# ywyue/AGILE3D

Measured on AMD Instinct MI355X. Metric: scenes/s (80k-voxel, 10 clicks), higher is better.
Workload: dtype f32; 1 GPU; batch of 16 synthetic 79736-voxel scenes, 10 clicks each (5 objects x 2), scene build + forward_backbone + 1 forward_mask per scene, fp32, eval; voxels=79736, queries=20, parallelism=scene-sharded x1 (no data-path collective), global_batch=16, steps_in_flight_per_gpu=4

## Files before the change

### agile3d_amd/csrc/spconv.hip

```cpp
#include "common.h"
#include <stdlib.h>

namespace a3d {

typedef float f32x4 __attribute__((ext_vector_type(4)));

struct ConvArgs {
  const float* in;
  int ldi, n_in;
  const int* nbr;
  int nbr_stride;
  const uint32_t* gmask;
  const float* w;
  int K, cin, cout;
  float* out;
  int ldo, n_out;
  const int* out_map;
  const float* scale;
  const float* shift;
  const float* res;
  int ldr;
  int relu;
  int zero_row;
  int tag_table, tag_level;
// ... 1071 lines not shown
  return A3D_OK;
}

template <int NS, int NCT, bool HAS2>
__global__ void __launch_bounds__(768) k_dense(const float* __restrict__ X, int ldx, const float* __restrict__ X2,
                                                   int ldx2, int n, const float* __restrict__ Wp,
                                                   const float* __restrict__ scale, const float* __restrict__ shift,
                                                   const float* __restrict__ res, int ldr, int relu,
                                                   float* __restrict__ Y, int ldy, int ngroups, int zero_row,
                                                   const int* __restrict__ out_map) {
  extern __shared__ __attribute__((aligned(16))) char smem[];
  f32x4* Wl = (f32x4*)smem;
  if (zero_row >= 0 && blockIdx.x == 0 && threadIdx.x < 16 * NCT) Y[(size_t)zero_row * ldy + threadIdx.x] = 0.f;
  const int lane = threadIdx.x & 63, wave = threadIdx.x >> 6;
  const int g = lane >> 4, j = lane & 15;
  const int nw = blockDim.x >> 6;
  const int stride = gridDim.x * nw;
  int grp = blockIdx.x * nw + wave;
  f32x4 nx[NS], nx2[HAS2 ? NS : 1];
  auto fetch = [&](int gq) {
    const int row = min(gq * 16 + j, n - 1);
    const float* xr = X + (size_t)row * ldx + 4 * g;
#pragma unroll
    for (int S = 0; S < NS; ++S) nx[S] = *(const f32x4*)(xr + 16 * S);
    if constexpr (HAS2) {
      const float* x2r = X2 + (size_t)row * ldx2 + 4 * g;
#pragma unroll
      for (int S = 0; S < NS; ++S) nx2[S] = *(const f32x4*)(x2r + 16 * S);
    }
  };
  if (grp < ngroups) fetch(grp);
  {
    constexpr int TOT = NS * NCT * 64;
    const int bd = blockDim.x;
    for (int base = threadIdx.x; base < TOT; base += 8 * bd) {
      f32x4 t8[8];
#pragma unroll
      for (int u = 0; u < 8; ++u)
        if (base + u * bd < TOT) t8[u] = ((const f32x4*)Wp)[base + u * bd];
#pragma unroll
      for (int u = 0; u < 8; ++u)
        if (base + u * bd < TOT) Wl[base + u * bd] = t8[u];
    }
  }
  __syncthreads();
  while (grp < ngroups) {
    f32x4 a[NS];
#pragma unroll
    for (int S = 0; S < NS; ++S) {
      if constexpr (HAS2) a[S] = nx[S] + nx2[S];
      else a[S] = nx[S];
    }
    const int next = grp + stride;
    if (next < ngroups) fetch(next);
    f32x4 acc[NCT];
#pragma unroll
    for (int ct = 0; ct < NCT; ++ct) acc[ct] = (f32x4){0.f, 0.f, 0.f, 0.f};
    {
      static_assert(NCT % 2 == 0, "pairs of 16-column tiles");
      constexpr int NP = NS * NCT / 2;
      const f32x4* Ws = Wl + lane;
      f32x4 c0 = Ws[0], c1 = Ws[64];
#pragma unroll
      for (int pi = 0; pi < NP; ++pi) {
        const int S = pi / (NCT / 2), ct = 2 * (pi % (NCT / 2));
        f32x4 n0 = c0, n1 = c1;
        if (pi + 1 < NP) {
          n0 = Ws[(2 * pi + 2) * 64];
          n1 = Ws[(2 * pi + 3) * 64];
        }
        __builtin_amdgcn_sched_barrier(0);
#pragma unroll
        for (int t = 0; t < 4; ++t) {
          acc[ct] = __builtin_amdgcn_mfma_f32_16x16x4f32(c0[t], a[S][t], acc[ct], 0, 0, 0);
          acc[ct + 1] = __builtin_amdgcn_mfma_f32_16x16x4f32(c1[t], a[S][t], acc[ct + 1], 0, 0, 0);
        }
        __builtin_amdgcn_sched_barrier(0);
        c0 = n0;
        c1 = n1;
      }
    }
    if (grp * 16 + j < n) {
      const int row = out_map ? out_map[grp * 16 + j] : grp * 16 + j;
#pragma unroll
      for (int ct = 0; ct < NCT; ++ct) {
        const int col = 16 * ct + 4 * g;
        f32x4 v = acc[ct];
        if (scale) v *= *(const f32x4*)(scale + col);
        if (shift) v += *(const f32x4*)(shift + col);
        if (res) v += *(const f32x4*)(res + (size_t)row * ldr + col);
        if (relu) {
#pragma unroll
          for (int t = 0; t < 4; ++t) v[t] = fmaxf(v[t], 0.f);
        }
        *(f32x4*)(Y + (size_t)row * ldy + col) = v;
      }
    }
    grp = next;
  }
}

static void allow_big_lds();
static bool dense_supported(int cin, int cout) {
  return (cin == 96 || cin == 128) && (cout == 96 || cout == 128);
}
static int launch_dense(const float* X, int ldx, const float* X2, int ldx2, int n, int cin, int cout, const float* Wp,
                        const float* scale, const float* shift, const float* res, int ldr, int relu, float* Y,
                        int ldy, int zero_row, int tag_level, const int* out_map, hipStream_t st) {
  if ((ldx | ldx2 | ldr | ldy) & 3) {
    set_error("a3d_linear: leading dimensions must be multiples of 4");
    return A3D_ERR_INVALID;
  }
  allow_big_lds();
  const int ngroups = (n + 15) / 16;
  const int nw = n >= 200000 ? 12 : 4, wg_per_cu = n >= 200000 ? 1 : 2;
  const size_t lds = (size_t)(cin / 16) * (cout / 16) * 1024;
  ProfScope ps(st, A3D_PROF_DENSE, 0, 1, cin, cout, n, A3D_OP_LINEAR, tag_level, 1);
  const int max_grid = 256 * wg_per_cu;
  const int grid = (ngroups + nw - 1) / nw < max_grid ? (ngroups + nw - 1) / nw : max_grid;
#define A3D_DENSE(NS_, NCT_) \
  do { \
    if (X2) k_dense<NS_, NCT_, true><<<grid, 64 * nw, lds, st>>>(X, ldx, X2, ldx2, n, Wp, scale, shift, res, ldr, relu, Y, ldy, ngroups, \
                                                                 zero_row, out_map); \
    else k_dense<NS_, NCT_, false><<<grid, 64 * nw, lds, st>>>(X, ldx, X2, ldx2, n, Wp, scale, shift, res, ldr, relu, Y, ldy, ngroups, \
                                                               zero_row, out_map); \
  } while (0)
  if (cin == 128 && cout == 128) A3D_DENSE(8, 8);
  else if (cin == 128 && cout == 96) A3D_DENSE(8, 6);
  else if (cin == 96 && cout == 128) A3D_DENSE(6, 8);
  else A3D_DENSE(6, 6);
#undef A3D_DENSE
  A3D_LAUNCH_CHECK();
  return A3D_OK;
}

template <int NT, int KS>
__global__ void __launch_bounds__(NT) k_stem(const int32_t* __restrict__ xyzb, int n,
                                              const uint64_t* __restrict__ hk, const int* __restrict__ hv,
                                              uint32_t hmask, const f32x4* __restrict__ feats4,
                                              const float* __restrict__ w, int ,
                                              const float* __restrict__ scale, const float* __restrict__ shift,
                                              int relu, float* out, int ldo, int zero_row, const Level glv) {
  extern __shared__ __attribute__((aligned(16))) char smem[];
  constexpr int ks = KS, K = KS * KS * KS;
  float* W = (float*)smem;
  int* nb = (int*)(W + K * 96);
  const int tid = threadIdx.x;
  for (int e = tid; e < K * 96; e += NT) W[e] = w[e];
  const int v0 = blockIdx.x * 64;
  const int h = ks / 2;
  constexpr int TPV = NT / 64, CPT = 32 / TPV;
  constexpr int SEG = (K + TPV - 1) / TPV;
  const int v = tid / TPV, cg = tid % TPV;
  const bool fused = glv.grid && n < (1 << 25);
  const int mrow = v0 + v;
  const int row = fused ? (mrow < n ? glv.perm[mrow] : n) : mrow;
  int mine[SEG];
  if (fused) {
    int4 c = (int4){0, 0, 0, 0};
    if (mrow < n) {
      int b_, X_, Y_, Z_;
      decode_key(glv.keys[mrow], 0, b_, X_, Y_, Z_);
      c = (int4){X_, Y_, Z_, b_};
    }
#pragma unroll
    for (int u = 0; u < SEG; ++u) {
      const int k = cg * SEG + u;
      mine[u] = -1;
      if (k < K && row < n)
        mine[u] = glv.grid[grid_cell(glv, c.w, c.x + (k % ks) - h, c.y + ((k / ks) % ks) - h, c.z + (k / (ks * ks)) - h)];
    }
  } else if (glv.grid) {
    for (int e0 = tid; e0 < 64 * K; e0 += 8 * NT) {
      int res[8];
#pragma unroll
      for (int u = 0; u < 8; ++u) {
        const int e = e0 + u * NT;
        const int vv = e / K, k = e - vv * K;
        const int rr = v0 + vv;
        res[u] = -1;
        if (e < 64 * K && rr < n) {
          const int4 c = *(const int4*)(xyzb + 4 * rr);
          res[u] = glv.grid[grid_cell(glv, c.w, c.x + (k % ks) - h, c.y + ((k / ks) % ks) - h, c.z + (k / (ks * ks)) - h)];
          if (res[u] >= 0) res[u] = glv.perm[res[u]];
        }
      }
#pragma unroll
      for (int u = 0; u < 8; ++u)
        if (e0 + u * NT < 64 * K) nb[e0 + u * NT] = res[u];
    }
  } else
  for (int e0 = tid; e0 < 64 * K; e0 += 4 * NT) {
    uint64_t key[4];
    uint32_t hh[4];
    int res[4];
    bool open[4];
#pragma unroll
    for (int u = 0; u < 4; ++u) {
      const int e = e0 + u * NT;
      const int v = e / K, k = e - v * K;
      const int row = v0 + v;
      res[u] = -1;
      open[u] = false;
      key[u] = 0;
      hh[u] = 0;
      if (e < 64 * K && row < n) {
        const int X = xyzb[4 * row + 0] + (k % ks) - h;
        const int Y = xyzb[4 * row + 1] + ((k / ks) % ks) - h;
        const int Z = xyzb[4 * row + 2] + (k / (ks * ks)) - h;
        const int b = xyzb[4 * row + 3];
        const int lim = kCoordOff;
        if (X >= -lim && X < lim && Y >= -lim && Y < lim && Z >= -lim && Z < lim) {
          key[u] = make_key(b, X, Y, Z, 0);
          hh[u] = hash64(key[u]) & hmask;
          open[u] = true;
        }
      }
    }
    for (uint32_t probe = 0; probe <= hmask; ++probe) {
      uint64_t got[4];
#pragma unroll
      for (int u = 0; u < 4; ++u) got[u] = open[u] ? hk[hh[u]] : kEmptyKey;
      bool any = false;
#pragma unroll
      for (int u = 0; u < 4; ++u) {
        if (!open[u]) continue;
        if (got[u] == key[u]) {
          res[u] = hv[hh[u]];
          open[u] = false;
        } else if (got[u] == kEmptyKey) {
          open[u] = false;
        } else {
          hh[u] = (hh[u] + 1) & hmask;
          any = true;
        }
      }
      if (!any) break;
    }
#pragma unroll
    for (int u = 0; u < 4; ++u)
      if (e0 + u * NT < 64 * K) nb[e0 + u * NT] = res[u];
  }
  __syncthreads();
  float acc[CPT];
#pragma unroll
  for (int c = 0; c < CPT; ++c) acc[c] = 0.f;
  if (n < (1 << 25)) {
    constexpr int seg = SEG;
    int cnt = 0;
#pragma unroll
    for (int u = 0; u < SEG; ++u) {
      const int k = cg * seg + u;
      if (!fused) mine[u] = k < K ? nb[v * K + k] : -1;
      cnt += mine[u] >= 0 ? 1 : 0;
    }
    int incl = cnt;
#pragma unroll
    for (int o = 1; o < TPV; o <<= 1) {
      const int t = __shfl_up(incl, o, 64);
      if (cg >= o) incl += t;
    }
    const int total = __shfl(incl, (threadIdx.x & 63) | (TPV - 1), 64);
    if (!fused) __syncthreads();
    int pos = incl - cnt;
#pragma unroll
    for (int u = 0; u < SEG; ++u)
      if (mine[u] >= 0) nb[v * K + pos++] = (int)((uint32_t)mine[u] | ((uint32_t)(cg * seg + u) << 25));
    __syncthreads();
    for (int i0 = 0; i0 < total; i0 += 8) {
      uint32_t e[8];
      f32x4 f[8];
#pragma unroll
      for (int u = 0; u < 8; ++u) e[u] = i0 + u < total ? (uint32_t)nb[v * K + i0 + u] : 0u;
#pragma unroll
      for (int u = 0; u < 8; ++u) f[u] = feats4[e[u] & 0x1ffffffu];
#pragma unroll
      for (int u = 0; u < 8; ++u) {
        if (i0 + u >= total) continue;
        const float* wk = W + (e[u] >> 25) * 96 + cg * CPT;
#pragma unroll
        for (int c = 0; c < CPT; ++c) acc[c] += f[u][0] * wk[c] + f[u][1] * wk[32 + c] + f[u][2] * wk[64 + c];
      }
    }
  } else
  for (int k0 = 0; k0 < K; k0 += 5) {
    int r[5];
    f32x4 f[5];
#pragma unroll
    for (int u = 0; u < 5; ++u) r[u] = k0 + u < K ? nb[v * K + k0 + u] : -1;
#pragma unroll
    for (int u = 0; u < 5; ++u) f[u] = feats4[r[u] >= 0 ? r[u] : 0];
#pragma unroll
    for (int u = 0; u < 5; ++u) {
      if (r[u] < 0) continue;
      const float* wk = W + (k0 + u) * 96 + cg * CPT;
#pragma unroll
      for (int c = 0; c < CPT; ++c) acc[c] += f[u][0] * wk[c] + f[u][1] * wk[32 + c] + f[u][2] * wk[64 + c];
    }
  }
  if (row < n) {
#pragma unroll
    for (int c = 0; c < CPT; ++c) {
      const int col = cg * CPT + c;
      float y = acc[c] * (scale ? scale[col] : 1.f) + (shift ? shift[col] : 0.f);
      if (relu) y = fmaxf(y, 0.f);
      out[(size_t)row * ldo + col] = y;
    }
  }
  if (zero_row >= 0 && blockIdx.x == 0 && tid < 32) out[(size_t)zero_row * ldo + tid] = 0.f;
}

__global__ void k_gather_feats(const float* __restrict__ feats3, const int* __restrict__ orig_row, int n,
                               f32x4* feats4, const int* __restrict__ perm) {
  const int f = blockIdx.x * blockDim.x + threadIdx.x;
  if (f >= n) return;
  const float* p = feats3 + (size_t)orig_row[perm ? perm[f] : f] * 3;
  feats4[f] = (f32x4){p[0], p[1], p[2], 0.f};
}

__global__ void k_pack_weight(const float* __restrict__ w, int K, int cin, int cout, float* out) {
  const size_t e = (size_t)blockIdx.x * blockDim.x + threadIdx.x;
  const size_t total = (size_t)K * cin * cout;
  if (e >= total) return;
  const int t = (int)(e & 3), lane = (int)((e >> 2) & 63);
  size_t rest = e >> 8;
  const int cout16 = cout >> 4, cin16 = cin >> 4;
  const int ct = (int)(rest % cout16);
  rest /= cout16;
  const int S = (int)(rest % cin16);
  const int k = (int)(rest / cin16);
  const int g = lane >> 4, j = lane & 15;
  out[e] = w[((size_t)k * cin + 16 * S + 4 * g + t) * cout + 16 * ct + j];
}

constexpr int kMaxQueuesPerOp = 1024;
constexpr int kSkMaxG = 1020;

struct SkPlan {
  int bn, ch, pair, nchunk, ov, n_cblk, G, ntile;
  size_t lds, slab_floats;
};
static int sk_ch(int cin, int bn) {
  if (bn == 128 && cin % 32 == 0) return 32;
  if (bn == 96 && cin % 32 == 0) return 32;
  const int cand[3] = {96, 64, 32};
  for (int i = 0; i < 3; ++i)
    if (cin % cand[i] == 0 && 2 * cand[i] * bn * 4 + 64 <= 80 * 1024) return cand[i];
  return 0;
}
static int sk_pair(int bn, int ch, int n_rows) {
  if (bn == 128) return ch == 32 && n_rows >= 8192;
  return bn == 96;
}
static int sk_wgs_per_cu(int bn, int ch, int pair, size_t lds) {
  int by_regs = 2;
  if (pair) {
    by_regs = (bn <= 96 && ch <= 32) ? 4 : 3;
  } else {
    if (bn == 32) by_regs = ch <= 32 ? 5 : 4;
    else if (bn == 64) by_regs = ch <= 32 ? 4 : 3;
    else if (bn == 96) by_regs = ch <= 48 ? 3 : 2;
  }
  const int by_lds = (int)(160 * 1024 / lds);
  const int w = by_regs < by_lds ? by_regs : by_lds;
  return w < 1 ? 1 : (w > 4 ? 4 : w);
}
static SkPlan plan_sk(int n_rows, int K, int cin, int cout, bool handoff, int force_ch = 0) {
  SkPlan p;
  p.ntile = (n_rows + 63) / 64;
  if (p.ntile < 1) p.ntile = 1;
  const int k_eff = K == 27 ? 13 : K;
  int gmax = 512;
  for (int pass = 0; pass < 2; ++pass) {
    p.bn = (cout % 128 == 0) ? 128 : cout;
    if (pass == 1 && cout % 64 == 0 && p.bn > 64) p.bn = 64;
    p.ch = force_ch > 0 && cin % force_ch == 0 ? force_ch : sk_ch(cin, p.bn);
    p.nchunk = p.ch ? cin / p.ch : 1;
    p.n_cblk = cout / p.bn;
    p.pair = sk_pair(p.bn, p.ch, n_rows);
    const int mfma_per_stage = p.ch / 4 * (p.bn / 16);
    p.ov = mfma_per_stage >= 128 ? 1 : mfma_per_stage >= 64 ? 2 : 3;
    p.lds = (size_t)2 * p.ch * p.bn * 4 + 64;
    gmax = 256 * sk_wgs_per_cu(p.bn, p.ch, p.pair, p.lds);
    if (gmax > kSkMaxG) gmax = kSkMaxG;
    const long long est = (long long)p.n_cblk * p.ntile * ((long long)p.nchunk * k_eff + p.ov);
    const int min_share = mfma_per_stage >= 128 ? 6 : 8;
    if (handoff) {
      long long G = est / min_share;
      const int small_share = 4;
      if (G < 256 && small_share < min_share) {
        G = est / small_share;
        if (G > 256) G = 256;
      }
      p.G = (int)(G < 1 ? 1 : (G > gmax ? gmax : G));
      p.slab_floats = (size_t)p.G * 64 * p.bn;
      if (p.G >= 256 || p.bn <= 64 || cout % 64) break;
    } else {
      const long long nu = (long long)p.n_cblk * p.ntile;
      p.G = (int)(nu < gmax ? nu : gmax);
      p.slab_floats = 0;
      break;
    }
  }
  return p;
}

struct DeepPlan {
  bool use;
  int bn, ch, P, G, n_cblk, ntile, nchunk, D;
  size_t lds, slab_floats;
  float est_us;
};
static int g_deep_mode = -1;
static int deep_mode() {
  if (g_deep_mode < 0) {
    const char* e = getenv("A3D_CONV_DEEP");
    g_deep_mode = e ? atoi(e) : 1;
  }
  return g_deep_mode;
}
static DeepPlan plan_deep(int n_rows, int K, int cin, int cout, int cin2, bool up = false) {
  DeepPlan best;
  memset(&best, 0, sizeof(best));
  if (!deep_mode() || K < 2 || K > 27 || cin % 32 || cout % 32) return best;
  static float max_us = -1.f;
  if (max_us < 0.f) {
    const char* e = getenv("A3D_DEEP_MAX_US");
    max_us = e ? (float)atof(e) : 23.f;
  }
  const int ntile = n_rows > 0 ? (n_rows + 63) / 64 : 1;
  const int k_eff = K == 27 ? (n_rows < 8000 ? 22 : n_rows < 32000 ? 17 : 14) : up ? 2 : K;
  static const int cand[5][2] = {{128, 32}, {64, 64}, {64, 32}, {32, 64}, {32, 32}};
  auto lds_of = [](int bn, int ch, int D) -> size_t { return (size_t)D * ((ch / 16) * (bn / 16) + 4 * (ch / 16)) * 1024 + 28 * 64 * 4 + 64; };
  float best_t = 1e30f;
  for (int ci = 0; ci < 5; ++ci) {
    const int bn = cand[ci][0], ch = cand[ci][1];
    if (cout % bn || cin % ch || (cin2 > 0 && cin2 % ch)) continue;
    const int units = cout / bn * ntile;
    if (units > kMaxQueuesPerOp - 2) continue;
    const int S = k_eff * (cin / ch) + (cin2 > 0 ? cin2 / ch : 0);
    const int ns = ch / 16, nct = bn / 16;
    const float mf = (float)ns * (float)nct * 0.0533f;
    const float tstage = (ns < 4 ? 0.45f : 0.3f) + 0.04f * (float)(ns + ns * nct / 4) + mf;
    if ((float)units * (float)S * mf / 256.f > max_us) continue;
    for (int D = 3; D >= 2; --D) {
      const int per_cu = 160 * 1024 / lds_of(bn, ch, D) >= 2 ? 2 : 1;
      if (D == 2 && (per_cu < 2 || 160 * 1024 / lds_of(bn, ch, 3) >= 2)) continue;
      for (int P = 1; P <= 24; ++P) {
        if (P > 1 && S / P < 2) break;
        const int G = units * P;
        if (G > 256 * per_cu) break;
        const int stages = (S + P - 1) / P;
        const float ts = G > 256 ? fmaxf(tstage + 0.1f, 2.2f * mf + 0.3f) : tstage + (D == 2 ? 0.05f : 0.f);
        const float t = 2.6f + (float)stages * ts + (P > 1 ? 1.0f + (float)P * (0.2f + 0.12f * bn / 32.f) * (G > 256 ? 1.5f : 1.f) : 0.f);
        if (t < best_t) {
          best_t = t;
          best.bn = bn, best.ch = ch, best.P = P, best.G = G, best.n_cblk = cout / bn, best.ntile = ntile, best.nchunk = cin / ch;
          best.D = D;
        }
// ... 342 lines not shown
  off += align256(pf * 4);
  L.queue_off = off;
  off += align256((size_t)(n_ops > 0 ? n_ops : 1) * kMaxQueuesPerOp * 4);
  L.total = off;
  return A3D_OK;
}

}

using namespace a3d;

extern "C" int a3d_pack_conv_weight(const float* w_dev, int kernel_volume, int cin, int cout,
                                    float* packed_dev, void* stream) {
  if (!w_dev || !packed_dev || kernel_volume < 1 || cin % 16 || cout % 16) {
    set_error("a3d_pack_conv_weight: bad arguments (K=%d cin=%d cout=%d)", kernel_volume, cin, cout);
    return A3D_ERR_INVALID;
  }
  const size_t total = (size_t)kernel_volume * cin * cout;
  k_pack_weight<<<(unsigned)((total + 255) / 256), 256, 0, (hipStream_t)stream>>>(w_dev, kernel_volume, cin, cout, packed_dev);
  A3D_LAUNCH_CHECK();
  return A3D_OK;
}

__global__ void __launch_bounds__(256) k_pack_weight_multi(const a3d_pack_job* __restrict__ tab, int nj) {
  int lo = 0, hi = nj;
  while (hi - lo > 1) {
    const int mid = (lo + hi) >> 1;
    if (tab[mid].chunk0 <= (int)blockIdx.x) lo = mid; else hi = mid;
  }
  const a3d_pack_job jb = tab[lo];
  const size_t total = (size_t)jb.K * jb.cin * jb.cout;
  const size_t base = (size_t)((int)blockIdx.x - jb.chunk0) * A3D_MT_CHUNK;
  const int cout16 = jb.cout >> 4, cin16 = jb.cin >> 4;
  for (int i = threadIdx.x; i < A3D_MT_CHUNK; i += 256) {
    const size_t e = base + i;
    if (e >= total) break;
    const int t = (int)(e & 3), lane = (int)((e >> 2) & 63);
    size_t rest = e >> 8;
    const int ct = (int)(rest % cout16);
    rest /= cout16;
    const int S = (int)(rest % cin16);
    const int k = (int)(rest / cin16);
    const int ci = 16 * S + 4 * (lane >> 4) + t, co = 16 * ct + (lane & 15);
    size_t si;
    if (jb.transposed) si = ((size_t)(jb.flip ? jb.K - 1 - k : k) * jb.src_cin + jb.c0 + co) * jb.src_cout + ci;
    else si = ((size_t)k * jb.src_cin + ci) * jb.src_cout + co;
    jb.dst[e] = jb.src[si];
  }
}

extern "C" int a3d_pack_conv_weights_multi(const a3d_pack_job* table_dev, int n_jobs, int64_t n_chunks, void* stream) {
  if (!table_dev || n_jobs < 1 || n_chunks < 1 || n_chunks > (int64_t)1 << 30) {
    set_error("a3d_pack_conv_weights_multi: bad arguments");
    return A3D_ERR_INVALID;
  }
  k_pack_weight_multi<<<(unsigned)n_chunks, 256, 0, (hipStream_t)stream>>>(table_dev, n_jobs);
  A3D_LAUNCH_CHECK();
  return A3D_OK;
}

extern "C" size_t a3d_conv_weight_packed_floats(int kernel_volume, int cin, int cout) {
  return (size_t)kernel_volume * cin * cout;
}

extern "C" size_t a3d_program_workspace_bytes(const a3d_scene* s, const a3d_buf_desc* bufs, int n_bufs,
                                              const a3d_op* ops, int n_ops) {
  ProgLayout L;
  if (layout_program(s, bufs, n_bufs, ops, n_ops, L) != A3D_OK) return 0;
  return L.total + 256;
}

extern "C" size_t a3d_program_buffer_offset(const a3d_scene* s, const a3d_buf_desc* bufs, int n_bufs, int i) {
  ProgLayout L;
  if (i < 0 || i >= n_bufs || layout_program(s, bufs, n_bufs, nullptr, 0, L) != A3D_OK) return (size_t)-1;
  return L.buf_off[i];
}

extern "C" int a3d_program_run(const a3d_scene* s, const a3d_buf_desc* bufs, int n_bufs, const a3d_op* ops,
                               int n_ops, const float* feats3_dev, float* ext_out_dev, int ext_out_ld,
                               void* workspace_dev, size_t workspace_bytes, void* stream) {
  ProgLayout L;
  int rc = layout_program(s, bufs, n_bufs, ops, n_ops, L);
  if (rc != A3D_OK) return rc;
  if (!workspace_dev || workspace_bytes < L.total || ((uintptr_t)workspace_dev & 255)) {
    set_error("a3d_program_run: workspace too small or misaligned (%zu < %zu)", workspace_bytes, L.total);
    return A3D_ERR_WORKSPACE;
  }
  hipStream_t st = (hipStream_t)stream;
  char* ws = (char*)workspace_dev;
  f32x4* feats4 = (f32x4*)(ws + L.feats4_off);
  float* partial = (float*)(ws + L.partial_off);
  int* queues = (int*)(ws + L.queue_off);
  A3D_HIP_CHECK(hipMemsetAsync(queues, 0, (size_t)n_ops * kMaxQueuesPerOp * 4, st));
  bool feats_ready = false;
  auto buf_ptr = [&](int id) -> float* { return (float*)(ws + L.buf_off[id]); };

  for (int i = 0; i < n_ops; ++i) {
    const a3d_op& o = ops[i];
    const int Lin = o.level_in;
    if (Lin < 0 || Lin >= A3D_NUM_LEVELS) {
      set_error("op %d: bad level", i);
      return A3D_ERR_INVALID;
    }
    float* out = nullptr;
    int ldo = 0;
    const int* out_map = nullptr;
    int zero_row = -1;
    int lvl_out = Lin;
    if (o.kind == A3D_OP_DOWN) lvl_out = Lin + 1;
    if (o.kind == A3D_OP_UP) lvl_out = Lin - 1;
    if (o.out_buf == A3D_BUF_EXT_OUT) {
      if (!ext_out_dev || lvl_out != 0 || o.kind == A3D_OP_UP) {
        set_error("op %d: external output needs a level-0, non-transposed op", i);
        return A3D_ERR_INVALID;
      }
      out = ext_out_dev + o.out_coff;
      ldo = ext_out_ld;
      out_map = s->orig_row;
    } else {
      if (o.out_buf < 0 || o.out_buf >= n_bufs || bufs[o.out_buf].level != lvl_out ||
          o.out_coff + o.cout > bufs[o.out_buf].channels) {
        set_error("op %d: bad output buffer", i);
        return A3D_ERR_INVALID;
      }
      out = buf_ptr(o.out_buf) + o.out_coff;
      ldo = bufs[o.out_buf].channels;
      zero_row = s->lv[lvl_out].n;
    }
    const float* res = nullptr;
    int ldr = 0;
    if (o.res_buf != A3D_BUF_NONE) {
      if (o.res_buf < 0 || o.res_buf >= n_bufs || bufs[o.res_buf].level != lvl_out ||
          o.res_coff + o.cout > bufs[o.res_buf].channels || o.out_buf == A3D_BUF_EXT_OUT) {
        set_error("op %d: bad residual buffer", i);
        return A3D_ERR_INVALID;
      }
      res = buf_ptr(o.res_buf) + o.res_coff;
      ldr = bufs[o.res_buf].channels;
    }

    if (o.kind == A3D_OP_STEM) {
      if (Lin != 0 || o.cin != 3 || o.cout != 32 || !feats3_dev ||
          !(o.kernel_volume == 125 || o.kernel_volume == 27)) {
        set_error("op %d: stem expects level 0, 3->32 channels, 5^3 or 3^3 kernel", i);
        return A3D_ERR_UNSUPPORTED;
      }
      const Level& lv = s->lv[0];
      const int ks = o.kernel_volume == 125 ? 5 : 3;
      const bool morton = lv.grid && ks / 2 <= kGridPad && lv.n < (1 << 25);
      if (!feats_ready) {
        k_gather_feats<<<(lv.n + 255) / 256, 256, 0, st>>>(feats3_dev, s->orig_row, lv.n, feats4, morton ? lv.perm : nullptr);
        feats_ready = true;
      }
      const size_t lds = (size_t)o.kernel_volume * 96 * 4 + (size_t)64 * o.kernel_volume * 4;
      ProfScope ps(st, A3D_PROF_STEM, 0, o.kernel_volume, 3, 32, lv.n);
      Level glv = lv;
      if (ks / 2 > kGridPad) glv.grid = nullptr;
      if (ks == 5)
        k_stem<512, 5><<<(lv.n + 63) / 64, 512, lds, st>>>(lv.xyzb, lv.n, lv.hkeys, lv.hvals, lv.hmask, feats4, o.w_dev, ks,
                                                           o.scale_dev, o.shift_dev, o.relu, out, ldo, zero_row, glv);
      else
        k_stem<512, 3><<<(lv.n + 63) / 64, 512, lds, st>>>(lv.xyzb, lv.n, lv.hkeys, lv.hvals, lv.hmask, feats4, o.w_dev, ks,
                                                           o.scale_dev, o.shift_dev, o.relu, out, ldo, zero_row, glv);
      A3D_LAUNCH_CHECK();
      continue;
    }

    if (o.in_buf < 0 || o.in_buf >= n_bufs || bufs[o.in_buf].level != Lin ||
        o.in_coff + o.cin > bufs[o.in_buf].channels) {
      set_error("op %d: bad input buffer", i);
      return A3D_ERR_INVALID;
    }
    ConvArgs a;
    memset(&a, 0, sizeof(a));
    a.in = buf_ptr(o.in_buf) + o.in_coff;
    a.ldi = bufs[o.in_buf].channels;
    a.n_in = s->lv[Lin].n;
    a.w = o.w_dev;
    a.K = o.kernel_volume;
    a.cin = o.cin;
    a.cout = o.cout;
    a.out = out;
    a.ldo = ldo;
    a.out_map = out_map;
    a.scale = o.scale_dev;
    a.shift = o.shift_dev;
    a.res = res;
    a.ldr = ldr;
    a.relu = o.relu;
    a.zero_row = zero_row;
    a.n_out = s->lv[lvl_out].n;
    a.tag_table = o.kind;
    a.tag_level = Lin;
    if (o.proj_cin > 0) {
      if (o.kind != A3D_OP_CONV3 || o.proj_buf < 0 || o.proj_buf >= n_bufs || bufs[o.proj_buf].level != Lin ||
          o.proj_coff + o.proj_cin > bufs[o.proj_buf].channels || o.scale_dev) {
        set_error("op %d: bad fused projection", i);
        return A3D_ERR_INVALID;
      }
      a.in2 = buf_ptr(o.proj_buf) + o.proj_coff;
      a.ldi2 = bufs[o.proj_buf].channels;
      a.cin2 = o.proj_cin;
    }
    const int* pre = nullptr;
    switch (o.kind) {
      case A3D_OP_CONV3:
        if (o.kernel_volume != 27) { set_error("op %d: CONV3 needs kernel volume 27", i); return A3D_ERR_INVALID; }
        a.nbr = s->lv[Lin].nbr27;
        a.nbr_stride = s->lv[Lin].npad;
        a.gmask = s->lv[Lin].gmask27;
        pre = s->lv[Lin].pre27;
        break;
      case A3D_OP_DOWN:
        if (o.kernel_volume != 8 || Lin >= A3D_NUM_LEVELS - 1) { set_error("op %d: bad DOWN", i); return A3D_ERR_INVALID; }
        a.nbr = s->lv[Lin].child8;
        a.nbr_stride = s->lv[Lin + 1].npad;
        a.gmask = s->lv[Lin].gmask_down;
        pre = s->lv[Lin].pre_down;
        break;
      case A3D_OP_UP:
        if (o.kernel_volume != 8 || Lin < 1) { set_error("op %d: bad UP", i); return A3D_ERR_INVALID; }
        a.nbr = s->lv[Lin - 1].up8;
        a.nbr_stride = s->lv[Lin - 1].npad;
        a.gmask = s->lv[Lin - 1].gmask_up;
        a.out_map = s->lv[Lin - 1].up_rows;
        pre = s->lv[Lin - 1].pre_up;
        break;
      case A3D_OP_LINEAR:
        if (o.kernel_volume != 1) { set_error("op %d: LINEAR needs kernel volume 1", i); return A3D_ERR_INVALID; }
        break;
      default:
        set_error("op %d: unknown kind %d", i, o.kind);
        return A3D_ERR_INVALID;
    }
    bool head_after = false;
    if (o.head_cout > 0) {
      if (!o.head_w_dev || !ext_out_dev || lvl_out != 0 || o.kind == A3D_OP_UP || o.out_buf == A3D_BUF_EXT_OUT ||
          o.head_cout % 16 || o.head_cout > ext_out_ld) {
        set_error("op %d: a fused head needs a level-0 op into a buffer, packed head weights and the external output", i);
        return A3D_ERR_INVALID;
      }
      bool handoff_h = o.kernel_volume > 1;
      if (handoff_h && o.kernel_volume <= 8) {
        const SkPlan q = plan_sk(a.n_out, a.K, a.cin, a.cout, false);
        if ((long long)q.ntile * q.n_cblk >= 192) handoff_h = false;
      }
      if (o.kind != A3D_OP_LINEAR && a.cin2 == 0 && !(conv_wl_supported(a)) && sk_head_ok(a.n_out, a.K, a.cin, a.cout, o.head_cout, handoff_h)) {
        a.head_w = o.head_w_dev;
        a.head_bias = o.head_bias_dev;
        a.head_out = ext_out_dev;
        a.head_ld = ext_out_ld;
        a.head_cout = o.head_cout;
        a.head_map = s->orig_row;
      } else {
        head_after = true;
      }
    }
    if (a.cin2 > 0 && !sk_fused_ok(a.n_out, a.cin, a.cout, a.cin2)) {
      ConvArgs c1 = a;
      c1.in2 = nullptr, c1.cin2 = 0, c1.ldi2 = 0, c1.relu = 0;
      rc = launch_conv_sk(c1, pre, partial, L.partial_floats, queues + (size_t)i * kMaxQueuesPerOp, st);
      if (rc != A3D_OK) return rc;
      if (a.out_map) {
        set_error("op %d: fused projection has no fallback for a row-mapped output", i);
        return A3D_ERR_UNSUPPORTED;
      }
      ConvArgs c2;
      memset(&c2, 0, sizeof(c2));
      c2.in = a.in2, c2.ldi = a.ldi2, c2.n_in = a.n_out, c2.K = 1, c2.cin = a.cin2, c2.cout = a.cout;
      c2.w = a.w + (size_t)27 * a.cin * a.cout;
      c2.out = a.out, c2.ldo = a.ldo, c2.n_out = a.n_out, c2.res = a.out, c2.ldr = a.ldo, c2.relu = a.relu;
      c2.zero_row = a.zero_row, c2.tag_table = A3D_OP_LINEAR, c2.tag_level = Lin;
      rc = launch_conv_sk(c2, nullptr, nullptr, 0, nullptr, st);
      if (rc != A3D_OK) return rc;
    } else
    if (o.kind == A3D_OP_LINEAR && dense_supported(a.cin, a.cout) && a.n_out >= 4096)
      rc = launch_dense(a.in, a.ldi, nullptr, 0, a.n_out, a.cin, a.cout, a.w, a.scale, a.shift, a.res, a.ldr, a.relu,
                        a.out, a.ldo, a.zero_row, Lin, a.out_map, st);
    else
      rc = launch_conv_sk(a, pre, partial, L.partial_floats, queues + (size_t)i * kMaxQueuesPerOp, st);
    if (rc != A3D_OK) return rc;
    if (head_after) {
      if (dense_supported(o.cout, o.head_cout) && a.n_out >= 4096)
        rc = launch_dense(out, ldo, nullptr, 0, a.n_out, o.cout, o.head_cout, o.head_w_dev, nullptr, o.head_bias_dev, nullptr, 0, 0,
                          ext_out_dev, ext_out_ld, -1, Lin, s->orig_row, st);
      else {
        ConvArgs h;
        memset(&h, 0, sizeof(h));
        h.in = out, h.ldi = ldo, h.n_in = a.n_out, h.w = o.head_w_dev, h.K = 1, h.cin = o.cout, h.cout = o.head_cout;
        h.out = ext_out_dev, h.ldo = ext_out_ld, h.n_out = a.n_out, h.out_map = s->orig_row, h.shift = o.head_bias_dev;
        h.zero_row = -1, h.tag_table = A3D_OP_LINEAR, h.tag_level = Lin;
        rc = launch_conv_sk(h, nullptr, nullptr, 0, nullptr, st);
      }
      if (rc != A3D_OK) return rc;
    }
  }
  return A3D_OK;
}

extern "C" size_t a3d_conv_apply_workspace_bytes(const a3d_scene* s, int kind, int level_in, int cin, int cout) {
  if (!s || level_in < 0 || level_in >= A3D_NUM_LEVELS) return 0;
  int lvl_out = level_in + (kind == A3D_OP_DOWN ? 1 : kind == A3D_OP_UP ? -1 : 0);
  if (lvl_out < 0 || lvl_out >= A3D_NUM_LEVELS) return 0;
  const int K = kind == A3D_OP_CONV3 ? 27 : kind == A3D_OP_LINEAR ? 1 : 8;
  SkPlan q = plan_sk(s->lv[lvl_out].n, K, cin, cout, true);
  size_t slab = q.slab_floats;
  const DeepPlan dp = plan_deep(s->lv[lvl_out].n, K, cin, cout, 0, kind == A3D_OP_UP);
  if (dp.use && dp.slab_floats > slab) slab = dp.slab_floats;
// ... 203 lines not shown
```

Baseline: 649.5 scenes/s.

## Add MFMA-based stem convolution kernel for Morton-ordered dense grid path

Adds a k_stem_mfma kernel that computes the 3->32 stem sparse convolution with fp32 16x16x4 MFMA instructions. Each wave handles 16 voxels and walks the kernel window as runs along x, packing contiguous x-neighbour features into the K dimension. It prefetches neighbour grid indices one z-slice ahead and skips runs the whole wave finds empty. The Morton path now dispatches to this kernel, and the old fused branch in k_stem is removed, adding kernel complexity and a packed LDS weight layout.

```diff
diff --git a/agile3d_amd/csrc/spconv.hip b/agile3d_amd/csrc/spconv.hip
--- a/agile3d_amd/csrc/spconv.hip
+++ b/agile3d_amd/csrc/spconv.hip
@@ -1247,25 +1247,9 @@
   constexpr int TPV = NT / 64, CPT = 32 / TPV;
   constexpr int SEG = (K + TPV - 1) / TPV;
   const int v = tid / TPV, cg = tid % TPV;
-  const bool fused = glv.grid && n < (1 << 25);
-  const int mrow = v0 + v;
-  const int row = fused ? (mrow < n ? glv.perm[mrow] : n) : mrow;
+  const int row = v0 + v;
   int mine[SEG];
-  if (fused) {
-    int4 c = (int4){0, 0, 0, 0};
-    if (mrow < n) {
-      int b_, X_, Y_, Z_;
-      decode_key(glv.keys[mrow], 0, b_, X_, Y_, Z_);
-      c = (int4){X_, Y_, Z_, b_};
-    }
-#pragma unroll
-    for (int u = 0; u < SEG; ++u) {
-      const int k = cg * SEG + u;
-      mine[u] = -1;
-      if (k < K && row < n)
-        mine[u] = glv.grid[grid_cell(glv, c.w, c.x + (k % ks) - h, c.y + ((k / ks) % ks) - h, c.z + (k / (ks * ks)) - h)];
-    }
-  } else if (glv.grid) {
+  if (glv.grid) {
     for (int e0 = tid; e0 < 64 * K; e0 += 8 * NT) {
       int res[8];
 #pragma unroll
@@ -1346,7 +1330,7 @@
 #pragma unroll
     for (int u = 0; u < SEG; ++u) {
       const int k = cg * seg + u;
-      if (!fused) mine[u] = k < K ? nb[v * K + k] : -1;
+      mine[u] = k < K ? nb[v * K + k] : -1;
       cnt += mine[u] >= 0 ? 1 : 0;
     }
     int incl = cnt;
@@ -1356,7 +1340,7 @@
       if (cg >= o) incl += t;
     }
     const int total = __shfl(incl, (threadIdx.x & 63) | (TPV - 1), 64);
-    if (!fused) __syncthreads();
+    __syncthreads();
     int pos = incl - cnt;
 #pragma unroll
     for (int u = 0; u < SEG; ++u)
@@ -1400,6 +1384,108 @@
       float y = acc[c] * (scale ? scale[col] : 1.f) + (shift ? shift[col] : 0.f);
       if (relu) y = fmaxf(y, 0.f);
       out[(size_t)row * ldo + col] = y;
+    }
+  }
+  if (zero_row >= 0 && blockIdx.x == 0 && tid < 32) out[(size_t)zero_row * ldo + tid] = 0.f;
+}
+
+template <int KS>
+__global__ void __launch_bounds__(512) k_stem_mfma(int n, const f32x4* __restrict__ feats4, const float* __restrict__ w,
+                                                   const float* __restrict__ scale, const float* __restrict__ shift, int relu,
+                                                   float* out, int ldo, int zero_row, int vec, const Level lv) {
+  extern __shared__ __attribute__((aligned(16))) char smem[];
+  constexpr int NRUN = KS * KS, NS = KS == 5 ? 4 : 3, H = KS / 2;
+  f32x4* Wf = (f32x4*)smem;
+  const int tid = threadIdx.x, lane = tid & 63, wave = tid >> 6, g = lane >> 4, j = lane & 15;
+  for (int e = tid; e < NRUN * 128; e += 512) {
+    const int gg = (e >> 4) & 3, co = 16 * ((e >> 6) & 1) + (e & 15), run = e >> 7;
+    f32x4 v = (f32x4){0.f, 0.f, 0.f, 0.f};
+#pragma unroll
+    for (int s = 0; s < 4; ++s) {
+      const int kk = 4 * gg + s;
+      const bool used = KS == 5 ? kk < 15 : (gg < 3 && s < 3);
+      const int cell = KS == 5 ? kk / 3 : gg, ci = KS == 5 ? kk % 3 : s;
+      if (used) v[s] = w[((run * KS + cell) * 3 + ci) * 32 + co];
+    }
+    Wf[e] = v;
+  }
+  __syncthreads();
+  const ptrdiff_t sy = lv.gdim[0], sz = (ptrdiff_t)lv.gdim[0] * lv.gdim[1];
+  const int cA = KS == 5 ? (g == 3 ? 4 : g) : g, cB = g + 1;
+  const bool hasA = KS == 5 || g < 3, hasB = KS == 5 && g < 3;
+  const bool o1 = g == 1, o2 = g == 2;
+  const int ngroups = (n + 15) >> 4;
+  for (int grp = blockIdx.x * 8 + wave; grp < ngroups; grp += gridDim.x * 8) {
+    const int mr = grp * 16 + j;
+    const bool ok = mr < n;
+    const int* gp = lv.grid;
+    if (ok) {
+      int b_, X_, Y_, Z_;
+      decode_key(lv.keys[mr], 0, b_, X_, Y_, Z_);
+      gp += grid_cell(lv, b_, X_ - H, Y_, Z_);
+    }
+    const int row = ok ? lv.perm[mr] : 0;
+    int nbA[KS], nbB[KS], nxA[KS], nxB[KS];
+#pragma unroll
+    for (int y = 0; y < KS; ++y) {
+      const ptrdiff_t o = -H * sz + (y - H) * sy;
+      nxA[y] = ok && hasA ? gp[o + cA] : -1;
+      nxB[y] = ok && hasB ? gp[o + cB] : -1;
+    }
+    f32x4 acc0 = (f32x4){0.f, 0.f, 0.f, 0.f}, acc1 = acc0;
+#pragma unroll
+    for (int z = 0; z < KS; ++z) {
+      f32x4 fa[KS], fb[KS];
+#pragma unroll
+      for (int y = 0; y < KS; ++y) {
+        nbA[y] = nxA[y];
+        nbB[y] = nxB[y];
+        fa[y] = nbA[y] >= 0 ? feats4[nbA[y]] : (f32x4){0.f, 0.f, 0.f, 0.f};
+        fb[y] = nbB[y] >= 0 ? feats4[nbB[y]] : (f32x4){0.f, 0.f, 0.f, 0.f};
+      }
+      if (z + 1 < KS) {
+#pragma unroll
+        for (int y = 0; y < KS; ++y) {
+          const ptrdiff_t o = (z + 1 - H) * sz + (y - H) * sy;
+          nxA[y] = ok && hasA ? gp[o + cA] : -1;
+          nxB[y] = ok && hasB ? gp[o + cB] : -1;
+        }
+      }
+#pragma unroll
+      for (int y = 0; y < KS; ++y) {
+        if (__ballot((nbA[y] & nbB[y]) >= 0) == 0) continue;
+        float b[4];
+        if (KS == 5) {
+          b[0] = o2 ? fa[y][2] : o1 ? fa[y][1] : fa[y][0];
+          b[1] = o2 ? fb[y][0] : o1 ? fa[y][2] : fa[y][1];
+          b[2] = o2 ? fb[y][1] : o1 ? fb[y][0] : fa[y][2];
+          b[3] = o2 ? fb[y][2] : o1 ? fb[y][1] : fb[y][0];
+        } else {
+          b[0] = fa[y][0], b[1] = fa[y][1], b[2] = fa[y][2], b[3] = 0.f;
+        }
+        const int run = z * KS + y;
+        const f32x4 a0 = Wf[(run * 2 + 0) * 64 + lane], a1 = Wf[(run * 2 + 1) * 64 + lane];
+#pragma unroll
+        for (int s = 0; s < NS; ++s) {
+          acc0 = __builtin_amdgcn_mfma_f32_16x16x4f32(a0[s], b[s], acc0, 0, 0, 0);
+          acc1 = __builtin_amdgcn_mfma_f32_16x16x4f32(a1[s], b[s], acc1, 0, 0, 0);
+        }
+      }
+    }
+    if (ok) {
+#pragma unroll
+      for (int mt = 0; mt < 2; ++mt) {
+        const int col = 16 * mt + 4 * g;
+        f32x4 y = mt ? acc1 : acc0;
+#pragma unroll
+        for (int r = 0; r < 4; ++r) {
+          y[r] = y[r] * (scale ? scale[col + r] : 1.f) + (shift ? shift[col + r] : 0.f);
+          if (relu) y[r] = fmaxf(y[r], 0.f);
+        }
+        float* p = out + (size_t)row * ldo + col;
+        if (vec) *(f32x4*)p = y;
+        else p[0] = y[0], p[1] = y[1], p[2] = y[2], p[3] = y[3];
+      }
     }
   }
   if (zero_row >= 0 && blockIdx.x == 0 && tid < 32) out[(size_t)zero_row * ldo + tid] = 0.f;
@@ -2048,8 +2134,19 @@
         k_gather_feats<<<(lv.n + 255) / 256, 256, 0, st>>>(feats3_dev, s->orig_row, lv.n, feats4, morton ? lv.perm : nullptr);
         feats_ready = true;
       }
+      ProfScope ps(st, A3D_PROF_STEM, 0, o.kernel_volume, 3, 32, lv.n);
+      if (morton) {
+        const size_t lds = (size_t)ks * ks * 2 * 64 * sizeof(f32x4);
+        const int want = (lv.n + 127) / 128, grid = want < 1 ? 1 : want < 512 ? want : 512;
+        const int vec = (((uintptr_t)out | ((uintptr_t)ldo * 4)) & 15) == 0;
+        if (ks == 5)
+          k_stem_mfma<5><<<grid, 512, lds, st>>>(lv.n, feats4, o.w_dev, o.scale_dev, o.shift_dev, o.relu, out, ldo, zero_row, vec, lv);
+        else
+          k_stem_mfma<3><<<grid, 512, lds, st>>>(lv.n, feats4, o.w_dev, o.scale_dev, o.shift_dev, o.relu, out, ldo, zero_row, vec, lv);
+        A3D_LAUNCH_CHECK();
+        continue;
+      }
       const size_t lds = (size_t)o.kernel_volume * 96 * 4 + (size_t)64 * o.kernel_volume * 4;
-      ProfScope ps(st, A3D_PROF_STEM, 0, o.kernel_volume, 3, 32, lv.n);
       Level glv = lv;
       if (ks / 2 > kGridPad) glv.grid = nullptr;
       if (ks == 5)
```

Result: no change. 655.8 scenes/s (median of 6 runs) (+1.0%).
